# z430/keyword-spotting

Hardware: AMD Instinct MI355X
Metric: 1s 16kHz clips/sec end-to-end (wav->label) (higher is better)
Workload: dtype f32

## Files before the change

### keyword-spotting_amd/csrc/kws_mfcc.hip

```cpp
#include <cstdlib>

#include "kws_augment_dev.h"
#include "kws_internal.h"
#include "kws_mfcc_dev.h"

namespace kws {
namespace {

template <typename T, bool TAIL6>
__device__ __forceinline__ void mfcc_body(const FrontendParams& p, const FrontendTables& t, const T* __restrict__ wav,
                                          float* __restrict__ out, const RefineList& rl) {
    extern __shared__ __attribute__((aligned(16))) unsigned char smem[];
    const int nfp = (p.nfilt + 3) & ~3;
    float* dctb = reinterpret_cast<float*>(smem);
    cf* tw2 = reinterpret_cast<cf*>(dctb + ((p.numcep * nfp + 3) & ~3));
    float* ybuf = reinterpret_cast<float*>(tw2 + 64);
    unsigned char* scr0 = reinterpret_cast<unsigned char*>(ybuf + ((p.chunk_samples + 7) & ~7));

    const int tid = threadIdx.x, lane = tid & 63, wv = tid >> 6;
    const int clip = blockIdx.y;
    const int f0 = blockIdx.x * MFCC_FRAMES_PER_WG;
    const T* __restrict__ x = wav + (size_t)clip * p.n_samples;

    const int s0 = f0 * p.frame_step;
// ... 76 lines not shown
            }
        } else {
#pragma unroll
            for (int n1 = 0; n1 < 8; ++n1) {
                const int i = 64 * n1 + lane;
                const bool in = i < p.frame_len;
                const float la = ya[i], lb = yb[i];
                const float a = in ? la : 0.f, b = (in && has_b) ? lb : 0.f;
                v[n1] = cf{a, b};
                ora |= __builtin_bit_cast(uint32_t, a);
                orb |= __builtin_bit_cast(uint32_t, b);
            }
        }
        const bool nza = __any((ora << 1) != 0u);
        const bool nzb = __any((orb << 1) != 0u);
        const uint32_t flags = mfcc_pair(v, nza, nzb, has_b, p, sc, t1, ml, lane,
                                         out + ((size_t)clip * p.num_frames + fa) * p.numcep,
                                         out + ((size_t)clip * p.num_frames + fa + 1) * p.numcep);
        if (flags && rl.ctr && lane == 0) {
            const unsigned long long old = atomicAdd(reinterpret_cast<unsigned long long*>(rl.ctr), 1ull | ((unsigned long long)__builtin_popcount(flags) << 32));
            const int at = (int)(unsigned)old;
            if (at < rl.cap) rl.list[at] = (int)((((unsigned)(rl.clip0 + clip) * (unsigned)((p.num_frames + 1) / 2) + (unsigned)(fa >> 1)) << 2) | flags);
        }
        wave_lds_order();
    }
}

#ifndef KWS_MFCC_EU
#define KWS_MFCC_EU 4
#endif
__global__ __launch_bounds__(MFCC_THREADS) __attribute__((amdgpu_waves_per_eu(KWS_MFCC_EU, KWS_MFCC_EU))) void kws_mfcc_i16_tile_kernel(FrontendParams p, FrontendTables t,
                                                                    const int16_t* __restrict__ wav,
                                                                    float* __restrict__ out, RefineList rl) {
    mfcc_body<int16_t, true>(p, t, wav, out, rl);
}
__global__ __launch_bounds__(MFCC_THREADS) __attribute__((amdgpu_waves_per_eu(KWS_MFCC_EU, KWS_MFCC_EU))) void kws_mfcc_f32_kernel(FrontendParams p, FrontendTables t,
                                                                    const float* __restrict__ wav,
                                                                    float* __restrict__ out, RefineList rl) {
    mfcc_body<float, true>(p, t, wav, out, rl);
}
__global__ __launch_bounds__(MFCC_THREADS) __attribute__((amdgpu_waves_per_eu(KWS_MFCC_EU, KWS_MFCC_EU))) void kws_mfcc_i16_any_kernel(FrontendParams p, FrontendTables t,
                                                                    const int16_t* __restrict__ wav,
                                                                    float* __restrict__ out, RefineList rl) {
    mfcc_body<int16_t, false>(p, t, wav, out, rl);
}
__global__ __launch_bounds__(MFCC_THREADS) __attribute__((amdgpu_waves_per_eu(KWS_MFCC_EU, KWS_MFCC_EU))) void kws_mfcc_f32_any_kernel(FrontendParams p, FrontendTables t,
                                                                    const float* __restrict__ wav,
                                                                    float* __restrict__ out, RefineList rl) {
    mfcc_body<float, false>(p, t, wav, out, rl);
}

constexpr int WR_PAIRS = 2, WR_FRAMES = 2 * WR_PAIRS;
constexpr int WR_SPAN = 1024;
constexpr int WR_WAVE_BYTES = WR_SPAN * 4 + SCR_BYTES;

typedef float float4_a4 __attribute__((ext_vector_type(4), aligned(4)));
__device__ __forceinline__ void aug_vec8(const AugClip& c, int n0, int n, float (&a)[8]) {
    if (n0 + 8 > n) {
#pragma unroll
        for (int i = 0; i < 8; ++i) a[i] = 0.f;
        return;
    }
    const int r = uniform_i(-c.shift & 7);
    const int base = n0 - c.shift - r;
    uint4 lo = make_uint4(0, 0, 0, 0), hi = lo;
    if (!c.silence) {
        if (base >= 0 && base + 8 <= n) lo = *reinterpret_cast<const uint4*>(c.x + base);
        if (base + 8 >= 0 && base + 16 <= n) hi = *reinterpret_cast<const uint4*>(c.x + base + 8);
    }
    const uint32_t w[8] = {lo.x, lo.y, lo.z, lo.w, hi.x, hi.y, hi.z, hi.w};
    const uint32_t m2 = (r & 4) ? ~0u : 0u, m1 = (r & 2) ? ~0u : 0u;
    uint32_t u[6], v[5];
#pragma unroll
    for (int k = 0; k < 6; ++k) u[k] = (w[k + 2] & m2) | (w[k] & ~m2);
#pragma unroll
    for (int k = 0; k < 5; ++k) v[k] = (u[k + 1] & m1) | (u[k] & ~m1);
#pragma unroll
    for (int k = 0; k < 4; ++k) {
        const uint32_t wd = (r & 1) ? __builtin_amdgcn_alignbyte(v[k + 1], v[k], 2) : v[k];
        a[2 * k] = pcm_unit((int16_t)(wd & 0xffffu));
        a[2 * k + 1] = pcm_unit((int16_t)(wd >> 16));
    }
    if (c.bg) {
        const int k0 = c.off + n0;
        float g[8];
        if (k0 >= 0 && k0 + 8 <= c.bg_len) {
            const float4_a4 g0 = *reinterpret_cast<const float4_a4*>(c.bg + k0);
            const float4_a4 g1 = *reinterpret_cast<const float4_a4*>(c.bg + k0 + 4);
            g[0] = g0.x, g[1] = g0.y, g[2] = g0.z, g[3] = g0.w, g[4] = g1.x, g[5] = g1.y, g[6] = g1.z, g[7] = g1.w;
        } else {
#pragma unroll
            for (int i = 0; i < 8; ++i) {
                const int k = c.off + n0 + i;
                g[i] = (k >= 0 && k < c.bg_len) ? c.bg[k] : 0.f;
            }
        }
#pragma unroll
        for (int i = 0; i < 8; ++i) a[i] = __fadd_rn(a[i], __fmul_rn(g[i], c.vol));
    }
}

__host__ __device__ inline size_t mfcc_wr_lds_bytes(const FrontendParams& p) {
    const int nfp = (p.nfilt + 3) & ~3;
    return sizeof(float) * (size_t)(((p.numcep * nfp + 3) & ~3) + 2 * 64) + (size_t)MFCC_WAVES * WR_WAVE_BYTES;
}

template <bool AUG>
__device__ __forceinline__ void mfcc_wr_body(FrontendParams p, FrontendTables t, const int16_t* __restrict__ wav,
                                             float* __restrict__ out, RefineList rl, int B, int chunks_per_wave,
                                             AugmentArgs aug) {
    extern __shared__ __attribute__((aligned(16))) unsigned char smem[];
    const int nfp = (p.nfilt + 3) & ~3;
    float* dctb = reinterpret_cast<float*>(smem);
    cf* tw2 = reinterpret_cast<cf*>(dctb + ((p.numcep * nfp + 3) & ~3));
    const int tid = threadIdx.x, lane = tid & 63, wv = tid >> 6;
    unsigned char* mine = reinterpret_cast<unsigned char*>(tw2 + 64) + wv * WR_WAVE_BYTES;
    float* ybuf = reinterpret_cast<float*>(mine);
    unsigned char* scr = mine + WR_SPAN * 4;

    for (int i = tid; i < (p.numcep * nfp + 3) / 4; i += MFCC_THREADS)
        reinterpret_cast<float4*>(dctb)[i] = reinterpret_cast<const float4*>(t.dct_pad)[i];
    fill_tw2(t.twiddle, tw2, tid);
    cf t1[8];
    load_twiddles(t.twiddle, lane, t1);
    MelLane ml;
    load_mel_lane(t, lane, ml);
    zero_scratch(scr, lane);

    const int n_chunks = (p.num_frames + WR_FRAMES - 1) / WR_FRAMES;
    const int waves_per_clip = (n_chunks + chunks_per_wave - 1) / chunks_per_wave;
    const int gw = blockIdx.x * MFCC_WAVES + wv;
    const int clip = gw / waves_per_clip, part = gw - clip * waves_per_clip;
    int c = part * chunks_per_wave;
    const int c_end = min(n_chunks, c + chunks_per_wave);
    const bool active = clip < B && c < c_end;
    const int16_t* __restrict__ x = AUG ? nullptr : wav + (size_t)(active ? clip : 0) * p.n_samples;
    AugClip ac{};
    if constexpr (AUG) ac = aug_clip(aug, active ? clip : 0, p.n_samples);
    const int chunk_step = WR_FRAMES * p.frame_step;

    uint4 v0 = make_uint4(0, 0, 0, 0), v1 = v0;
    int16_t before = 0;
    auto fetch = [&](int cc) {
        const int s0 = cc * chunk_step;
        const int n0 = s0 + 8 * lane, n1 = n0 + 512;
        v0 = n0 + 8 <= p.n_samples ? *reinterpret_cast<const uint4*>(x + n0) : make_uint4(0, 0, 0, 0);
        v1 = n1 + 8 <= p.n_samples ? *reinterpret_cast<const uint4*>(x + n1) : make_uint4(0, 0, 0, 0);
        before = s0 > 0 ? x[s0 - 1] : (int16_t)0;
    };
    (void)fetch;
#ifdef KWS_X_MFCC_PREFETCH
    if (!AUG && active) fetch(c);
#endif
    __syncthreads();
    if (!active) return;

    const PairScratch sc = {reinterpret_cast<cf*>(scr + SCR_XBUF), reinterpret_cast<float2*>(scr + SCR_PBUF),
                            reinterpret_cast<float*>(scr + SCR_LBUF), dctb, tw2, nfp};
    const float pre = p.preemph;
    uint32_t fmask = 0u;
    int pair0 = 2 * c;
#define KWS_FLUSH_FLAGS()                                                                                                          \
    if (fmask && rl.ctr) {                                                                                                          \
        const int lane = (int)__builtin_amdgcn_mbcnt_hi(~0u, __builtin_amdgcn_mbcnt_lo(~0u, 0u));  \
        const uint32_t fk = lane < 16 ? (fmask >> (2 * lane)) & 3u : 0u;                                                            \
        const uint32_t has = (uint32_t)__ballot(fk != 0u);                                                                          \
        unsigned long long old = 0ull;                                                                                              \
        if (lane == 0)                                                                                                              \
            old = atomicAdd(reinterpret_cast<unsigned long long*>(rl.ctr),                                                          \
                            (unsigned long long)__builtin_popcount(has) | ((unsigned long long)__builtin_popcount(fmask) << 32));   \
        const int at = __builtin_amdgcn_readfirstlane((int)(unsigned)old) + __builtin_popcount(has & ((1u << (lane & 31)) - 1u));   \
        if (fk != 0u && at < rl.cap)                                                                                                \
            rl.list[at] = (int)((((unsigned)(rl.clip0 + clip) * (unsigned)((p.num_frames + 1) / 2) + (unsigned)(pair0 + lane)) << 2) | fk); \
    }
    for (; c < c_end; ++c) {
#ifndef KWS_X_MFCC_PREFETCH
        if constexpr (!AUG) fetch(c);
#endif
        if constexpr (AUG) {
            const int s0 = c * chunk_step;
            float a0[8], a1[8];
            aug_vec8(ac, s0 + 8 * lane, p.n_samples, a0);
            aug_vec8(ac, s0 + 512 + 8 * lane, p.n_samples, a1);
            const float w0 = __int_as_float(__builtin_amdgcn_update_dpp(0, __float_as_int(a0[7]), 0x138, 0xf, 0xf, false));
            const float w1 = __int_as_float(__builtin_amdgcn_update_dpp(0, __float_as_int(a1[7]), 0x138, 0xf, 0xf, false));
            const float last0 = __int_as_float(__builtin_amdgcn_readlane(__float_as_int(a0[7]), 63));
            const float before_a = s0 > 0 ? aug_sample(ac, s0 - 1, p.n_samples) : 0.f;
            auto emphasise = [&](const float (&a)[8], float prev, int n, float* dst) {
                float y[8];
#pragma unroll
                for (int i = 0; i < 8; ++i) {
                    y[i] = __fsub_rn(a[i], __fmul_rn(pre, prev));
                    prev = a[i];
                }
                if (n == 0) y[0] = a[0];
                if (n + 8 > p.n_samples) {
#pragma unroll
                    for (int i = 0; i < 8; ++i) y[i] = 0.f;
                }
                reinterpret_cast<float4*>(dst)[0] = make_float4(y[0], y[1], y[2], y[3]);
                reinterpret_cast<float4*>(dst)[1] = make_float4(y[4], y[5], y[6], y[7]);
            };
            emphasise(a0, lane == 0 ? before_a : w0, s0 + 8 * lane, ybuf + 8 * lane);
            emphasise(a1, lane == 0 ? last0 : w1, s0 + 512 + 8 * lane, ybuf + 512 + 8 * lane);
        } else {
            const int s0 = c * chunk_step;
            const uint32_t w0 = (uint32_t)__builtin_amdgcn_update_dpp(0, (int)v0.w, 0x138, 0xf, 0xf, false);
            const uint32_t w1 = (uint32_t)__builtin_amdgcn_update_dpp(0, (int)v1.w, 0x138, 0xf, 0xf, false);
            const uint32_t last0 = (uint32_t)__builtin_amdgcn_readlane((int)v0.w, 63);
            float prev0 = lane == 0 ? to_unit(before) : to_unit((int16_t)(w0 >> 16));
            float prev1 = lane == 0 ? to_unit((int16_t)(last0 >> 16)) : to_unit((int16_t)(w1 >> 16));
            auto convert = [&](const uint4& raw, float prev, int n, float* dst) {
                const uint32_t wd[4] = {raw.x, raw.y, raw.z, raw.w};
                float y[8];
#pragma unroll
                for (int i = 0; i < 8; ++i) {
                    const float cur = to_unit((int16_t)((wd[i >> 1] >> (16 * (i & 1))) & 0xffffu));
                    y[i] = __fsub_rn(cur, __fmul_rn(pre, prev));
                    prev = cur;
                }
                if (n == 0) y[0] = to_unit((int16_t)(wd[0] & 0xffffu));
                if (n + 8 > p.n_samples) {
#pragma unroll
                    for (int i = 0; i < 8; ++i) y[i] = 0.f;
                }
                reinterpret_cast<float4*>(dst)[0] = make_float4(y[0], y[1], y[2], y[3]);
                reinterpret_cast<float4*>(dst)[1] = make_float4(y[4], y[5], y[6], y[7]);
            };
            convert(v0, prev0, s0 + 8 * lane, ybuf + 8 * lane);
            convert(v1, prev1, s0 + 512 + 8 * lane, ybuf + 512 + 8 * lane);
        }
        wave_lds_order();
#ifdef KWS_X_MFCC_PREFETCH
        if (!AUG && c + 1 < c_end) fetch(c + 1);
#endif
#pragma unroll 1
        for (int pr = 0; pr < WR_PAIRS; ++pr) {
            const int fa = WR_FRAMES * c + 2 * pr;
            if (fa >= p.num_frames) break;
            const bool has_b = fa + 1 < p.num_frames;
            const float* ya = ybuf + (2 * pr) * p.frame_step;
            const float* yb = ya + p.frame_step;
            cf v[8];
            uint32_t ora = 0u, orb = 0u;
#pragma unroll
            for (int n1 = 0; n1 < 7; ++n1) {
                const int i = 64 * n1 + lane;
                float a = ya[i], b = yb[i];
                if (n1 == 6) {
                    const bool in = i < p.frame_len;
                    a = in ? a : 0.f, b = in ? b : 0.f;
                }
                v[n1] = cf{a, b};
                ora |= __builtin_bit_cast(uint32_t, a);
                orb |= __builtin_bit_cast(uint32_t, b);
            }
            v[7] = cf{0.f, 0.f};
            if (!has_b) {
#pragma unroll
                for (int n1 = 0; n1 < 7; ++n1) v[n1].y = 0.f;
                orb = 0u;
            }
            const bool nza = __any((ora << 1) != 0u);
            const bool nzb = __any((orb << 1) != 0u);
            const uint32_t flags = mfcc_pair(v, nza, nzb, has_b, p, sc, t1, ml, lane,
                                             out + ((size_t)clip * p.num_frames + fa) * p.numcep,
                                             out + ((size_t)clip * p.num_frames + fa + 1) * p.numcep);
            fmask |= flags << (2 * ((fa >> 1) - pair0));
            wave_lds_order();
        }
        if (2 * (c + 1) - pair0 >= 16) {
            KWS_FLUSH_FLAGS()
            fmask = 0u;
            pair0 = 2 * (c + 1);
        }
    }
    KWS_FLUSH_FLAGS()
#undef KWS_FLUSH_FLAGS
}

__global__ __launch_bounds__(MFCC_THREADS) __attribute__((amdgpu_waves_per_eu(KWS_MFCC_EU, KWS_MFCC_EU))) void kws_mfcc_i16_kernel(
    FrontendParams p, FrontendTables t, const int16_t* __restrict__ wav, float* __restrict__ out, RefineList rl, int B, int chunks_per_wave) {
    mfcc_wr_body<false>(p, t, wav, out, rl, B, chunks_per_wave, AugmentArgs{});
}
#ifndef KWS_MFCC_AUG_EU
#define KWS_MFCC_AUG_EU 4
#endif
__global__ __launch_bounds__(MFCC_THREADS) __attribute__((amdgpu_waves_per_eu(KWS_MFCC_AUG_EU, KWS_MFCC_AUG_EU))) void kws_mfcc_augment_i16_kernel(
    FrontendParams p, FrontendTables t, AugmentArgs aug, float* __restrict__ out, RefineList rl, int B, int chunks_per_wave) {
    mfcc_wr_body<true>(p, t, nullptr, out, rl, B, chunks_per_wave, aug);
}

__global__ void kws_preemphasis_f32_kernel(const float* __restrict__ in, int n, float coeff, float* __restrict__ out) {
    for (int i = blockIdx.x * blockDim.x + threadIdx.x; i < n; i += gridDim.x * blockDim.x)
        out[i] = (i > 0) ? __fsub_rn(in[i], __fmul_rn(coeff, in[i - 1])) : in[i];
}

__global__ void kws_framesig_f32_kernel(const float* __restrict__ in, int n, int frame_len, int frame_step,
                                        int num_frames, const float* __restrict__ window,
                                        float* __restrict__ frames) {
    const long total = (long)num_frames * frame_len;
    for (long idx = blockIdx.x * (long)blockDim.x + threadIdx.x; idx < total; idx += (long)gridDim.x * blockDim.x) {
        const int f = (int)(idx / frame_len), i = (int)(idx % frame_len);
        const long s = (long)f * frame_step + i;
        float v = (s < n) ? in[s] : 0.f;
        if (window) v *= window[i];
        frames[idx] = v;
    }
}

__global__ __launch_bounds__(64) void kws_spec512_f32_kernel(FrontendTables t, const float* __restrict__ frames,
                                                             int num_frames, int frame_len, int power,
                                                             float* __restrict__ spec) {
    __shared__ __attribute__((aligned(16))) unsigned char smem[SCR_BYTES + 512];
    cf* xbuf = reinterpret_cast<cf*>(smem + SCR_XBUF);
    float2* pbuf = reinterpret_cast<float2*>(smem + SCR_PBUF);
    cf* tw2 = reinterpret_cast<cf*>(smem + SCR_BYTES);
    const int lane = threadIdx.x;
    const int fa = 2 * blockIdx.x;
    const bool has_b = fa + 1 < num_frames;
    cf t1[8];
    load_twiddles(t.twiddle, lane, t1);
    fill_tw2(t.twiddle, tw2, lane);
    wave_lds_order();
    const float* ya = frames + (size_t)fa * frame_len;
    const float* yb = ya + frame_len;
    cf v[8];
    bool nza = false, nzb = false;
#pragma unroll
    for (int n1 = 0; n1 < 8; ++n1) {
        const int i = 64 * n1 + lane;
        const bool in = i < frame_len;
        v[n1].x = in ? ya[i] : 0.f;
        v[n1].y = (in && has_b) ? yb[i] : 0.f;
        nza |= v[n1].x != 0.f;
        nzb |= v[n1].y != 0.f;
    }
    nza = __any(nza);
    nzb = __any(nzb);
    const PairLevel lv = equalise_levels(v);
    fft512(v, xbuf, t1, tw2, lane);
    float ea, eb;
    const int ident[4] = {lane, lane + 64, lane + 128, lane + 192};
// ... 70 lines not shown
    float vol = 0.f;
    if (d.n_files > 0 && (d.use_background || sil)) {
        const int k = draw_below(w[1], d.n_files);
        const int room = d.bg_len[k] - d.n_samples;
        off = d.bg_start[k] + (room > 0 ? draw_below(w[2], room) : 0);
        const float u = draw_unit(w[3]);
        if (sil)
            vol = u;
        else if (u < d.bg_frequency)
            vol = __fmul_rn(__fdiv_rn(u, d.bg_frequency), d.bg_volume);
    }
    d.bg_off[b] = off;
    d.bg_vol[b] = vol;
    d.silence[b] = sil ? 1 : 0;
}

}

hipError_t launch_augment_draw(hipStream_t s, const DrawArgs& d, int B) {
    hipLaunchKernelGGL(kws_augment_draw_kernel, dim3((B + 255) / 256), dim3(256), 0, s, d, B);
    return hipGetLastError();
}

size_t mfcc_lds_bytes(const FrontendParams& p) {
    const int nfp = (p.nfilt + 3) & ~3;
    return sizeof(float) * (size_t)(((p.numcep * nfp + 3) & ~3) + 2 * 64 + ((p.chunk_samples + 7) & ~7)) +
           (size_t)MFCC_WAVES * SCR_BYTES;
}

template <typename T, typename K>
static hipError_t launch_mfcc_t(K kernel, hipStream_t s, const FrontendParams& p, const FrontendTables& t, const T* d_wav,
                                int B, float* d_out, RefineList rl) {
    dim3 grid((p.num_frames + MFCC_FRAMES_PER_WG - 1) / MFCC_FRAMES_PER_WG, B);
    const size_t lds = mfcc_lds_bytes(p);
    if (lds > 64 * 1024) {
        hipError_t e = hipFuncSetAttribute(reinterpret_cast<const void*>(kernel), hipFuncAttributeMaxDynamicSharedMemorySize, (int)lds);
        if (e != hipSuccess) return e;
    }
    for (int b0 = 0; b0 < B; b0 += 65535) {
        const int nb = (B - b0 < 65535) ? (B - b0) : 65535;
        grid.y = nb;
        rl.clip0 = b0;
        hipLaunchKernelGGL(kernel, grid, dim3(MFCC_THREADS), lds, s, p, t, d_wav + (size_t)b0 * p.n_samples,
                           d_out + (size_t)b0 * p.num_frames * p.numcep, rl);
    }
    return hipGetLastError();
}

bool mfcc_wave_resident_ok(const FrontendParams& p) {
    const bool tail6 = p.frame_len > 384 && p.frame_len <= 448;
    return tail6 && p.vec_ok && (WR_FRAMES * p.frame_step) % 8 == 0 && (WR_FRAMES - 1) * p.frame_step + 448 <= WR_SPAN;
}

static int mfcc_wr_chunks_per_wave(int nb, int n_chunks) {
    int wpc = (n_chunks + 2) / 5;
    wpc = wpc < 1 ? 1 : wpc;
    int cpw = (n_chunks + wpc - 1) / wpc;
    const int fill = (int)(((long)nb * n_chunks + 4095) / 4096);
    cpw = cpw > fill ? (fill < 1 ? 1 : fill) : cpw;
    static const int cpw_env = [] {
        const char* e = getenv("KWS_X_MFCC_CPW");
        return e ? atoi(e) : 0;
    }();
    if (cpw_env > 0) cpw = cpw_env > 16 ? 16 : cpw_env;
    return cpw;
}

hipError_t launch_mfcc_flag(hipStream_t s, const FrontendParams& p, const FrontendTables& t, const int16_t* d_wav, int B,
                            float* d_out, const RefineList& rl) {
    const bool tail6 = p.frame_len > 384 && p.frame_len <= 448;
#ifndef KWS_X_MFCC_TILE_KERNEL
    if (mfcc_wave_resident_ok(p)) {
        const size_t lds = mfcc_wr_lds_bytes(p);
        const int n_chunks = (p.num_frames + WR_FRAMES - 1) / WR_FRAMES;
        for (int b0 = 0; b0 < B; b0 += (1 << 20)) {
            const int nb = B - b0 < (1 << 20) ? B - b0 : (1 << 20);
            const int cpw = mfcc_wr_chunks_per_wave(nb, n_chunks);
            const int waves_per_clip = (n_chunks + cpw - 1) / cpw;
            const long waves = (long)nb * waves_per_clip;
            RefineList r = rl;
            r.clip0 = b0;
            hipLaunchKernelGGL(kws_mfcc_i16_kernel, dim3((unsigned)((waves + MFCC_WAVES - 1) / MFCC_WAVES)), dim3(MFCC_THREADS), lds, s, p, t,
                               d_wav + (size_t)b0 * p.n_samples, d_out + (size_t)b0 * p.num_frames * p.numcep, r, nb, cpw);
        }
        return hipGetLastError();
    }
#endif
    return launch_mfcc_t(tail6 ? kws_mfcc_i16_tile_kernel : kws_mfcc_i16_any_kernel, s, p, t, d_wav, B, d_out, rl);
}

hipError_t launch_mfcc_augment_flag(hipStream_t s, const FrontendParams& p, const FrontendTables& t, const AugmentArgs& a, int B,
                                    float* d_out, const RefineList& rl) {
    if (!mfcc_wave_resident_ok(p)) return hipErrorInvalidValue;
    const size_t lds = mfcc_wr_lds_bytes(p);
    const int n_chunks = (p.num_frames + WR_FRAMES - 1) / WR_FRAMES;
    for (int b0 = 0; b0 < B; b0 += (1 << 20)) {
        const int nb = B - b0 < (1 << 20) ? B - b0 : (1 << 20);
        const int cpw = mfcc_wr_chunks_per_wave(nb, n_chunks);
        const int waves_per_clip = (n_chunks + cpw - 1) / cpw;
        const long waves = (long)nb * waves_per_clip;
        RefineList r = rl;
        r.clip0 = b0;
        AugmentArgs ab = a;
        ab.index += b0;
        if (ab.shift) ab.shift += b0;
        if (ab.bg_off) ab.bg_off += b0;
        if (ab.bg_vol) ab.bg_vol += b0;
        if (ab.silence) ab.silence += b0;
        hipLaunchKernelGGL(kws_mfcc_augment_i16_kernel, dim3((unsigned)((waves + MFCC_WAVES - 1) / MFCC_WAVES)), dim3(MFCC_THREADS), lds, s, p,
                           t, ab, d_out + (size_t)b0 * p.num_frames * p.numcep, r, nb, cpw);
    }
    return hipGetLastError();
}
hipError_t launch_mfcc_f32_flag(hipStream_t s, const FrontendParams& p, const FrontendTables& t, const float* d_wav, int B,
                                float* d_out, const RefineList& rl) {
    const bool tail6 = p.frame_len > 384 && p.frame_len <= 448;
    return launch_mfcc_t(tail6 ? kws_mfcc_f32_kernel : kws_mfcc_f32_any_kernel, s, p, t, d_wav, B, d_out, rl);
}
hipError_t launch_mfcc(hipStream_t s, const FrontendParams& p, const FrontendTables& t, const int16_t* d_wav, int B,
                       float* d_out) {
    return launch_mfcc_flag(s, p, t, d_wav, B, d_out, RefineList{});
}
hipError_t launch_mfcc_f32(hipStream_t s, const FrontendParams& p, const FrontendTables& t, const float* d_wav, int B,
                           float* d_out) {
    return launch_mfcc_f32_flag(s, p, t, d_wav, B, d_out, RefineList{});
}

hipError_t launch_stream_frame(hipStream_t s, const FrontendParams& p, const FrontendTables& t, const int16_t* d_hop,
                               int n_streams, int16_t* d_pcm_ring, int ring_len, float* d_feat_ring, int* d_hops, int* d_refine_ctr) {
    const size_t lds = stream_frame_lds_bytes(p);
    hipLaunchKernelGGL(kws_stream_frame_kernel, dim3((n_streams + 1) / 2), dim3(64), lds, s, p, t, d_hop, n_streams,
                       d_pcm_ring, ring_len, d_feat_ring, d_hops, d_refine_ctr);
    return hipGetLastError();
}

// ... 39 lines not shown
```

### keyword-spotting_amd/csrc/kws_mfcc_dev.h

```cpp
#pragma once
#include "kws_internal.h"
#include "kws_mfcc_f64_dev.h"

namespace kws {
namespace {

typedef float cf __attribute__((ext_vector_type(2)));

__device__ __forceinline__ cf cadd(cf a, cf b) { return a + b; }
__device__ __forceinline__ cf csub(cf a, cf b) { return a - b; }
__device__ __forceinline__ cf cmul(cf a, cf b) {
    cf t, r;
    asm("v_pk_mul_f32 %0, %1, %2 op_sel:[1,1] op_sel_hi:[1,0] neg_lo:[0,1]" : "=v"(t) : "v"(a), "v"(b));
    asm("v_pk_fma_f32 %0, %1, %2, %3 op_sel_hi:[0,1,1]" : "=v"(r) : "v"(a), "v"(b), "v"(t));
    return r;
}
__device__ __forceinline__ cf add_mi(cf a, cf b) {
    cf r;
    asm("v_pk_add_f32 %0, %1, %2 op_sel:[0,1] op_sel_hi:[1,0] neg_hi:[0,1]" : "=v"(r) : "v"(a), "v"(b));
    return r;
}
__device__ __forceinline__ cf sub_mi(cf a, cf b) {
    cf r;
    asm("v_pk_add_f32 %0, %1, %2 op_sel:[0,1] op_sel_hi:[1,0] neg_lo:[0,1]" : "=v"(r) : "v"(a), "v"(b));
// ... 335 lines not shown
        KWS_DPP_STEP("row_shr:2 row_mask:0xf bank_mask:0xf bound_ctrl:1")
        KWS_DPP_STEP("row_shr:4 row_mask:0xf bank_mask:0xf bound_ctrl:1")
        KWS_DPP_STEP("row_shr:8 row_mask:0xf bank_mask:0xf bound_ctrl:1")
        KWS_DPP_STEP("row_bcast:15 row_mask:0xa bank_mask:0xf")
        KWS_DPP_STEP("row_bcast:31 row_mask:0xc bank_mask:0xf")
        "s_nop 0"
        : "+v"(a), "+v"(b), "+v"(ma), "+v"(mb));
#undef KWS_DPP_STEP
    a = __builtin_bit_cast(float, __builtin_amdgcn_readlane(__builtin_bit_cast(int, a), 63));
    b = __builtin_bit_cast(float, __builtin_amdgcn_readlane(__builtin_bit_cast(int, b), 63));
    ma = __builtin_bit_cast(float, __builtin_amdgcn_readlane(__builtin_bit_cast(int, ma), 63));
    mb = __builtin_bit_cast(float, __builtin_amdgcn_readlane(__builtin_bit_cast(int, mb), 63));
}

template <bool FULL>
__device__ __forceinline__ unsigned long long peak_over(float v, float lim) {
    float mn = v;
#define KWS_MM_STEP(ctrl)                                      \
    "v_min_f32_dpp %0, %0, %0 " ctrl "\n\t"                    \
    "s_nop 1\n\t"
    asm("s_nop 1\n\t"
        KWS_MM_STEP("row_shr:1 row_mask:0xf bank_mask:0xf")
        KWS_MM_STEP("row_shr:2 row_mask:0xf bank_mask:0xf")
        KWS_MM_STEP("row_shr:4 row_mask:0xf bank_mask:0xf")
        KWS_MM_STEP("row_shr:8 row_mask:0xf bank_mask:0xf")
        "v_min_f32_dpp %0, %0, %0 row_bcast:15 row_mask:0xa bank_mask:0xf"
        : "+v"(mn));
    if constexpr (FULL)
        asm("s_nop 1\n\t"
            "v_min_f32_dpp %0, %0, %0 row_bcast:31 row_mask:0xc bank_mask:0xf"
            : "+v"(mn));
#undef KWS_MM_STEP
    return __ballot(mn < lim);
}
__device__ __forceinline__ void peak_over2(float va, float vb, float lim_a, float lim_b, bool& over_a, bool& over_b) {
    float a = va, b = vb;
#define KWS_MM_STEP(ctrl)                                      \
    "v_min_f32_dpp %0, %0, %0 " ctrl "\n\t"                    \
    "v_min_f32_dpp %1, %1, %1 " ctrl "\n\t"                    \
    "s_nop 0\n\t"
    asm("s_nop 1\n\t"
        KWS_MM_STEP("row_shr:1 row_mask:0xf bank_mask:0xf")
        KWS_MM_STEP("row_shr:2 row_mask:0xf bank_mask:0xf")
        KWS_MM_STEP("row_shr:4 row_mask:0xf bank_mask:0xf")
        KWS_MM_STEP("row_shr:8 row_mask:0xf bank_mask:0xf")
        KWS_MM_STEP("row_bcast:15 row_mask:0xa bank_mask:0xf")
        KWS_MM_STEP("row_bcast:31 row_mask:0xc bank_mask:0xf")
        : "+v"(a), "+v"(b));
#undef KWS_MM_STEP
    over_a = (__ballot(a < lim_a) >> 63) & 1ull;
    over_b = (__ballot(b < lim_b) >> 63) & 1ull;
}

__device__ __forceinline__ uint32_t mfcc_pair(cf (&v)[8], bool nza, bool nzb, bool has_b, const FrontendParams& p,
                                          const PairScratch& sc, const cf (&t1)[8], const MelLane& ml, int lane,
                                          float* __restrict__ out_a, float* __restrict__ out_b,
                                          float* lds_out_a = nullptr) {
    cf* xbuf = sc.xbuf;
    float2* pbuf = sc.pbuf;
    float* lbuf = sc.lbuf;
    const float* dctb = sc.dctb;
    const cf* tw2 = sc.tw2;
    const uint32_t gth = ml.gth;
    const int nfp = sc.nfp;
    const PairLevel lv = equalise_levels(v);
#if !defined(KWS_X_MFCC_STOP) || KWS_X_MFCC_STOP >= 1
    fft512(v, xbuf, t1, tw2, lane);
#endif
#if defined(KWS_X_MFCC_STOP) && KWS_X_MFCC_STOP <= 1
    if (lane < p.numcep) out_a[lane] = v[0].x + v[1].y + v[2].x + v[3].y + v[4].x + v[5].y + v[6].x + v[7].y + lv.pow_a;
    return 0u;
#endif

    float ea, eb, pka = 0.f, pkb = 0.f;
    if (p.refine_span > 0.f) {
        split_power(v, xbuf, pbuf, lane, 1, nza, nzb, ml.pslot, -1, lv, ea, eb, &pka, &pkb);
        wave_sum2_max2(ea, eb, pka, pkb);
    } else {
        split_power(v, xbuf, pbuf, lane, 1, nza, nzb, ml.pslot, -1, lv, ea, eb);
        wave_sum2(ea, eb);
    }
#if defined(KWS_X_MFCC_STOP) && KWS_X_MFCC_STOP == 2
    if (lane < p.numcep) out_a[lane] = ea + eb + pbuf[lane].x;
    return 0u;
#endif

    float ra = 0.f, fa_ = 0.f, rb = 0.f, fb_ = 0.f;
    {
        const float4* pc = reinterpret_cast<const float4*>(pbuf + lane * MEL_STRIDE);
#pragma unroll
        for (int h = 0; h < MEL_CHUNK / 2; ++h) {
            const float4 pw = pc[h];
            ra = fmaf(ml.rw[2 * h], pw.x, ra);
            fa_ = fmaf(ml.fw[2 * h], pw.x, fa_);
            rb = fmaf(ml.rw[2 * h], pw.y, rb);
            fb_ = fmaf(ml.fw[2 * h], pw.y, fb_);
            ra = fmaf(ml.rw[2 * h + 1], pw.z, ra);
            fa_ = fmaf(ml.fw[2 * h + 1], pw.z, fa_);
            rb = fmaf(ml.rw[2 * h + 1], pw.w, rb);
            fb_ = fmaf(ml.fw[2 * h + 1], pw.w, fb_);
        }
    }
    segment_suffix_sums(ra, fa_, rb, fb_, ml);
    float ma, mb;
    uint32_t flags = 0u;
    {
        const int r0 = gth & 255, nr = (gth >> 8) & 255, q0 = (gth >> 16) & 255, nq = gth >> 24;
        const float gra = __builtin_bit_cast(float, __builtin_amdgcn_ds_bpermute(4 * r0, __builtin_bit_cast(int, ra)));
        const float grb = __builtin_bit_cast(float, __builtin_amdgcn_ds_bpermute(4 * r0, __builtin_bit_cast(int, rb)));
        const float gfa = __builtin_bit_cast(float, __builtin_amdgcn_ds_bpermute(4 * q0, __builtin_bit_cast(int, fa_)));
        const float gfb = __builtin_bit_cast(float, __builtin_amdgcn_ds_bpermute(4 * q0, __builtin_bit_cast(int, fb_)));
        const float sa = (nr ? gra : 0.f) + (nq ? gfa : 0.f);
        const float sb = (nr ? grb : 0.f) + (nq ? gfb : 0.f);
        if (p.nfilt <= 32) {
            const auto sw = __builtin_amdgcn_permlane32_swap(__builtin_bit_cast(unsigned, sa), __builtin_bit_cast(unsigned, sb), false, false);
            const float s = __builtin_bit_cast(float, (unsigned)sw[0]);
            const float l = logf(s == 0.f ? PSF_EPS : s);
            ma = __builtin_bit_cast(float, __builtin_amdgcn_readlane(__builtin_bit_cast(int, l), 0));
            mb = __builtin_bit_cast(float, __builtin_amdgcn_readlane(__builtin_bit_cast(int, l), 32));
#if defined(KWS_X_MFCC_STOP) && KWS_X_MFCC_STOP == 3
            if (lane < p.numcep) out_a[lane] = l + ea + eb;
            return 0u;
#endif
            const int f = lane >> 5, j = lane & 31;
            const float cv = j < p.nfilt ? l - (f ? mb : ma) : 0.f;
            lbuf[64 * f + j] = cv;
            if (p.refine_span > 0.f) {
                const float lim = 0.6931471806f * __builtin_amdgcn_logf(f ? pkb : pka) - (f ? mb : ma) - p.refine_span;
                const unsigned long long over = peak_over<false>(cv, lim);
                flags = (uint32_t)((over >> 31) & 1u) | ((uint32_t)((over >> 63) & 1u) << 1);
            }
        } else {
            const float la = logf(sa == 0.f ? PSF_EPS : sa), lb = logf(sb == 0.f ? PSF_EPS : sb);
            ma = __builtin_bit_cast(float, __builtin_amdgcn_readfirstlane(__builtin_bit_cast(int, la)));
            mb = __builtin_bit_cast(float, __builtin_amdgcn_readfirstlane(__builtin_bit_cast(int, lb)));
            const float cva = lane < p.nfilt ? la - ma : 0.f, cvb = lane < p.nfilt ? lb - mb : 0.f;
            lbuf[lane] = cva;
            lbuf[64 + lane] = cvb;
            if (p.refine_span > 0.f) {
                bool oa, ob;
                peak_over2(cva, cvb, 0.6931471806f * __builtin_amdgcn_logf(pka) - ma - p.refine_span, 0.6931471806f * __builtin_amdgcn_logf(pkb) - mb - p.refine_span, oa, ob);
                flags = (uint32_t)oa | ((uint32_t)ob << 1);
            }
        }
    }
    wave_lds_order();

    {
        const int f = lane >> 5, i = lane & 31;
        if (i < p.numcep && (f == 0 || has_b)) {
            const float4* L4 = reinterpret_cast<const float4*>(lbuf + 64 * f);
            const float4* D4 = reinterpret_cast<const float4*>(dctb + i * nfp);
            float acc = 0.f;
            if (nfp == 28) {
#pragma unroll
                for (int j0 = 0; j0 < 7; j0 += 4) {
                    float4 d[4], l[4];
#pragma unroll
                    for (int j = 0; j < 4; ++j)
                        if (j0 + j < 7) d[j] = D4[j0 + j], l[j] = L4[j0 + j];
#pragma unroll
                    for (int j = 0; j < 4; ++j)
                        if (j0 + j < 7) {
                            acc = fmaf(d[j].x, l[j].x, acc);
                            acc = fmaf(d[j].y, l[j].y, acc);
                            acc = fmaf(d[j].z, l[j].z, acc);
                            acc = fmaf(d[j].w, l[j].w, acc);
                        }
                    __builtin_amdgcn_sched_barrier(0);
                }
            } else {
                for (int j = 0; j < nfp / 4; ++j) {
                    const float4 d = D4[j], l = L4[j];
                    acc = fmaf(d.x, l.x, acc);
                    acc = fmaf(d.y, l.y, acc);
                    acc = fmaf(d.z, l.z, acc);
                    acc = fmaf(d.w, l.w, acc);
                }
            }
            if (i == 0) {
                if (p.append_energy) {
                    const float e = f ? eb : ea;
                    acc = logf(e == 0.f ? PSF_EPS : e);
                } else {
                    float dsum = 0.f;
                    for (int j = 0; j < p.nfilt; ++j) dsum += dctb[j];
                    acc = fmaf(f ? mb : ma, dsum, acc);
                }
            }
            (f ? out_b : out_a)[i] = acc;
            if (lds_out_a && f == 0) lds_out_a[i] = acc;
        }
    }
    wave_lds_order();
    return has_b ? flags : (flags & 1u);
}


constexpr int STREAM_F64_BYTES = 16 * NFFT + 8 * 128;
__host__ __device__ __forceinline__ size_t stream_frame_lds_bytes(const FrontendParams& p) {
    const int nfp = (p.nfilt + 3) & ~3;
    return sizeof(float) * (size_t)(((p.numcep * nfp + 3) & ~3) + 2 * 64) + SCR_BYTES + STREAM_F64_BYTES;
}

template <typename F>
__device__ __forceinline__ void f64_redo_frame(const FrontendParams& p, const FrontendTables& t, d2* X, double* L, F&& get,
                                               float* __restrict__ out, float* lds_out, int lane) {
    bool nz = false;
#pragma unroll
    for (int n1 = 0; n1 < 8; ++n1) {
        const int i = 64 * n1 + lane;
        const float y = i < p.frame_len ? get(i) : 0.f;
        nz |= y != 0.f;
        X[sw512(i)] = d2{(double)y, 0.0};
    }
    nz = __any(nz);
    wave_order();
    spectrum_pair<true, NFFT>(X, X, reinterpret_cast<const d2*>(t.tw64), NFFT, 9, p.frame_len, 1.0 / (double)NFFT, lane);
    const F64Tabs tb = {reinterpret_cast<const d2*>(t.tw64), t.mel_w64, t.dct64, t.mel_edges};
    f64_tail<NBINS>(p, tb, NBINS, X, L, nz, false, false, out, out, lds_out, lane);
}
__device__ __forceinline__ long stream_frame_wave(const FrontendParams& p, const FrontendTables& t,
                                                  const int16_t* __restrict__ hop, int sa, int sb, bool has_b,
                                                  int16_t* __restrict__ pcm_ring, int ring_len,
                                                  float* __restrict__ feat_ring, int hops, unsigned char* smem, int lane,
                                                  float* lds_out_a, int* refine_ctr = nullptr) {
    const int nfp = (p.nfilt + 3) & ~3;
    float* dctb = reinterpret_cast<float*>(smem);
    cf* tw2 = reinterpret_cast<cf*>(dctb + ((p.numcep * nfp + 3) & ~3));
    unsigned char* scr = reinterpret_cast<unsigned char*>(tw2 + 64);
    const int step = p.frame_step;
    const long base = (long)step * hops;

    {
        const int n4 = (p.numcep * nfp + 3) / 4;
        const float4* src = reinterpret_cast<const float4*>(t.dct_pad);
        for (int i0 = 0; i0 < n4; i0 += 128) {
            const int i = i0 + lane, j = i + 64;
            const float4 a = i < n4 ? src[i] : make_float4(0.f, 0.f, 0.f, 0.f);
// ... 113 lines not shown
```

Measured before the change: 7.082 million.

## Specialise MFCC kernel for reference geometry and add optional global-to-LDS chunk DMA

Adds a REF template specialisation that hardcodes frame length, step, filter count and cepstral count for the standard 400/160/26/10 geometry, chosen at launch by a host check. This lets the compiler fold constants and drop runtime branches. It also adds an asynchronous global_load_lds prefetch path that pulls the next chunk's PCM into LDS while the current pair is computed. That path is compiled only when KWS_X_MFCC_CHUNK_DMA is defined, so by default only the specialisation runs. The per-wave LDS buffer layout changes, which may affect occupancy.

```diff
diff --git a/keyword-spotting_amd/csrc/kws_mfcc.hip b/keyword-spotting_amd/csrc/kws_mfcc.hip
--- a/keyword-spotting_amd/csrc/kws_mfcc.hip
+++ b/keyword-spotting_amd/csrc/kws_mfcc.hip
@@ -152,7 +152,20 @@
 
 constexpr int WR_PAIRS = 2, WR_FRAMES = 2 * WR_PAIRS;
 constexpr int WR_SPAN = 1024;
-constexpr int WR_WAVE_BYTES = WR_SPAN * 4 + SCR_BYTES;
+constexpr int WR_DMA_V1_BYTE = 3712, WR_DMA_V1_LANES = 46;
+constexpr int WR_YBUF_BYTES = WR_DMA_V1_BYTE + 16 * WR_DMA_V1_LANES;
+constexpr int WR_WAVE_BYTES = WR_YBUF_BYTES + SCR_BYTES;
+static_assert(WR_YBUF_BYTES >= WR_SPAN * 4, "the converted span (two float4 pairs per lane) lies inside the span buffer");
+static_assert(WR_DMA_V1_BYTE % 16 == 0 && WR_YBUF_BYTES % 16 == 0 && WR_WAVE_BYTES % 16 == 0 && SCR_BYTES % 16 == 0,
+              "both DMA regions and the scratch behind them start on 16 bytes in every wavefront");
+static_assert(WR_DMA_V1_BYTE + 16 * 64 <= WR_WAVE_BYTES, "the 16-byte read-back of every lane stays inside the wavefront's own LDS");
+static_assert(4 * (10 * 28 + 2 * 64) + MFCC_WAVES * WR_WAVE_BYTES <= 40960, "four workgroups per CU at the reference geometry (160 KiB of LDS)");
+
+__device__ __forceinline__ void glds16(const void* base, uint32_t byte_off, uint32_t lds_base) {
+    uint32_t keep;
+    asm volatile("s_nop 4\n\ts_mov_b32 %0, m0\n\ts_mov_b32 m0, %3\n\ts_nop 0\n\tglobal_load_lds_dwordx4 %1, %2\n\ts_mov_b32 m0, %0"
+                 : "=&s"(keep) : "v"(byte_off), "s"(base), "s"(lds_base) : "memory");
+}
 
 typedef float float4_a4 __attribute__((ext_vector_type(4), aligned(4)));
 __device__ __forceinline__ void aug_vec8(const AugClip& c, int n0, int n, float (&a)[8]) {
@@ -205,20 +218,20 @@
     return sizeof(float) * (size_t)(((p.numcep * nfp + 3) & ~3) + 2 * 64) + (size_t)MFCC_WAVES * WR_WAVE_BYTES;
 }
 
-template <bool AUG>
+template <bool AUG, bool REF>
 __device__ __forceinline__ void mfcc_wr_body(FrontendParams p, FrontendTables t, const int16_t* __restrict__ wav,
                                              float* __restrict__ out, RefineList rl, int B, int chunks_per_wave,
                                              AugmentArgs aug) {
     extern __shared__ __attribute__((aligned(16))) unsigned char smem[];
-    const int nfp = (p.nfilt + 3) & ~3;
+    const int nfp = REF ? 28 : (p.nfilt + 3) & ~3, dct_floats = REF ? 10 * 28 : p.numcep * nfp;
     float* dctb = reinterpret_cast<float*>(smem);
-    cf* tw2 = reinterpret_cast<cf*>(dctb + ((p.numcep * nfp + 3) & ~3));
-    const int tid = threadIdx.x, lane = tid & 63, wv = tid >> 6;
+    cf* tw2 = reinterpret_cast<cf*>(dctb + ((dct_floats + 3) & ~3));
+    const int tid = threadIdx.x, lane = tid & 63, wv = AUG ? tid >> 6 : __builtin_amdgcn_readfirstlane(tid >> 6);
     unsigned char* mine = reinterpret_cast<unsigned char*>(tw2 + 64) + wv * WR_WAVE_BYTES;
     float* ybuf = reinterpret_cast<float*>(mine);
-    unsigned char* scr = mine + WR_SPAN * 4;
-
-    for (int i = tid; i < (p.numcep * nfp + 3) / 4; i += MFCC_THREADS)
+    unsigned char* scr = mine + WR_YBUF_BYTES;
+
+    for (int i = tid; i < (dct_floats + 3) / 4; i += MFCC_THREADS)
         reinterpret_cast<float4*>(dctb)[i] = reinterpret_cast<const float4*>(t.dct_pad)[i];
     fill_tw2(t.twiddle, tw2, tid);
     cf t1[8];
@@ -234,10 +247,21 @@
     int c = part * chunks_per_wave;
     const int c_end = min(n_chunks, c + chunks_per_wave);
     const bool active = clip < B && c < c_end;
+#ifdef KWS_X_MFCC_HOT_PCM
+    const int16_t* __restrict__ x = wav;
+#else
     const int16_t* __restrict__ x = AUG ? nullptr : wav + (size_t)(active ? clip : 0) * p.n_samples;
+#endif
     AugClip ac{};
     if constexpr (AUG) ac = aug_clip(aug, active ? clip : 0, p.n_samples);
-    const int chunk_step = WR_FRAMES * p.frame_step;
+    const int frame_step = REF ? 160 : p.frame_step, frame_len = REF ? 400 : p.frame_len;
+    const int chunk_step = WR_FRAMES * frame_step;
+#if !defined(KWS_X_MFCC_CHUNK_DMA) || defined(KWS_X_MFCC_PREFETCH)
+    const bool dma = false;
+#else
+    const bool dma = !AUG && (REF || (8 * frame_step >= 16 * 64 && 4 * (3 * frame_step + 448) <= WR_DMA_V1_BYTE &&
+                                      3 * frame_step + frame_len <= 512 + 8 * WR_DMA_V1_LANES));
+#endif
 
     uint4 v0 = make_uint4(0, 0, 0, 0), v1 = v0;
     int16_t before = 0;
@@ -249,6 +273,27 @@
         before = s0 > 0 ? x[s0 - 1] : (int16_t)0;
     };
     (void)fetch;
+    const int c_first = c;
+    int16_t carried = 0;
+    auto dma_issue = [&](int cc) {
+        const int s0 = cc * chunk_step;
+        const int n0 = s0 + 8 * lane, n1 = n0 + 512;
+        const uint32_t base = (uint32_t)__builtin_amdgcn_readfirstlane((int)lds_addr(mine));
+#ifndef KWS_X_MFCC_DMA_DRY
+        if (n0 + 8 <= p.n_samples) glds16(x, 2u * (uint32_t)n0, base);
+        if (lane < WR_DMA_V1_LANES && n1 + 8 <= p.n_samples) glds16(x, 2u * (uint32_t)n1, base + WR_DMA_V1_BYTE);
+#endif
+    };
+    auto dma_take = [&](int cc) {
+        const int s0 = cc * chunk_step;
+        const int n0 = s0 + 8 * lane, n1 = n0 + 512;
+        asm volatile("s_waitcnt vmcnt(0)" ::: "memory");
+        const uint4 r0 = *reinterpret_cast<const uint4*>(mine + 16 * lane);
+        const uint4 r1 = *reinterpret_cast<const uint4*>(mine + WR_DMA_V1_BYTE + 16 * lane);
+        v0 = n0 + 8 <= p.n_samples ? r0 : make_uint4(0, 0, 0, 0);
+        v1 = lane < WR_DMA_V1_LANES && n1 + 8 <= p.n_samples ? r1 : make_uint4(0, 0, 0, 0);
+        before = carried;
+    };
 #ifdef KWS_X_MFCC_PREFETCH
     if (!AUG && active) fetch(c);
 #endif
@@ -275,7 +320,10 @@
     }
     for (; c < c_end; ++c) {
 #ifndef KWS_X_MFCC_PREFETCH
-        if constexpr (!AUG) fetch(c);
+        if constexpr (!AUG) {
+            if (dma && c != c_first) dma_take(c);
+            else fetch(c);
+        }
 #endif
         if constexpr (AUG) {
             const int s0 = c * chunk_step;
@@ -327,6 +375,7 @@
                 reinterpret_cast<float4*>(dst)[0] = make_float4(y[0], y[1], y[2], y[3]);
                 reinterpret_cast<float4*>(dst)[1] = make_float4(y[4], y[5], y[6], y[7]);
             };
+            if (dma) carried = (int16_t)((uint32_t)__builtin_amdgcn_readlane((int)v1.w, 15) >> 16);
             convert(v0, prev0, s0 + 8 * lane, ybuf + 8 * lane);
             convert(v1, prev1, s0 + 512 + 8 * lane, ybuf + 512 + 8 * lane);
         }
@@ -339,8 +388,8 @@
             const int fa = WR_FRAMES * c + 2 * pr;
             if (fa >= p.num_frames) break;
             const bool has_b = fa + 1 < p.num_frames;
-            const float* ya = ybuf + (2 * pr) * p.frame_step;
-            const float* yb = ya + p.frame_step;
+            const float* ya = ybuf + (2 * pr) * frame_step;
+            const float* yb = ya + frame_step;
             cf v[8];
             uint32_t ora = 0u, orb = 0u;
 #pragma unroll
@@ -348,7 +397,7 @@
                 const int i = 64 * n1 + lane;
                 float a = ya[i], b = yb[i];
                 if (n1 == 6) {
-                    const bool in = i < p.frame_len;
+                    const bool in = i < frame_len;
                     a = in ? a : 0.f, b = in ? b : 0.f;
                 }
                 v[n1] = cf{a, b};
@@ -363,11 +412,13 @@
             }
             const bool nza = __any((ora << 1) != 0u);
             const bool nzb = __any((orb << 1) != 0u);
-            const uint32_t flags = mfcc_pair(v, nza, nzb, has_b, p, sc, t1, ml, lane,
-                                             out + ((size_t)clip * p.num_frames + fa) * p.numcep,
-                                             out + ((size_t)clip * p.num_frames + fa + 1) * p.numcep);
+            const int numcep = REF ? 10 : p.numcep;
+            const uint32_t flags = mfcc_pair<REF>(v, nza, nzb, has_b, p, sc, t1, ml, lane,
+                                                  out + ((size_t)clip * p.num_frames + fa) * numcep,
+                                                  out + ((size_t)clip * p.num_frames + fa + 1) * numcep);
             fmask |= flags << (2 * ((fa >> 1) - pair0));
             wave_lds_order();
+            if (!AUG && dma && pr == 0 && c + 1 < c_end) dma_issue(c + 1);
         }
         if (2 * (c + 1) - pair0 >= 16) {
             KWS_FLUSH_FLAGS()
@@ -381,14 +432,18 @@
 
 __global__ __launch_bounds__(MFCC_THREADS) __attribute__((amdgpu_waves_per_eu(KWS_MFCC_EU, KWS_MFCC_EU))) void kws_mfcc_i16_kernel(
     FrontendParams p, FrontendTables t, const int16_t* __restrict__ wav, float* __restrict__ out, RefineList rl, int B, int chunks_per_wave) {
-    mfcc_wr_body<false>(p, t, wav, out, rl, B, chunks_per_wave, AugmentArgs{});
+    mfcc_wr_body<false, true>(p, t, wav, out, rl, B, chunks_per_wave, AugmentArgs{});
+}
+__global__ __launch_bounds__(MFCC_THREADS) __attribute__((amdgpu_waves_per_eu(KWS_MFCC_EU, KWS_MFCC_EU))) void kws_mfcc_i16_general_kernel(
+    FrontendParams p, FrontendTables t, const int16_t* __restrict__ wav, float* __restrict__ out, RefineList rl, int B, int chunks_per_wave) {
+    mfcc_wr_body<false, false>(p, t, wav, out, rl, B, chunks_per_wave, AugmentArgs{});
 }
 #ifndef KWS_MFCC_AUG_EU
 #define KWS_MFCC_AUG_EU 4
 #endif
 __global__ __launch_bounds__(MFCC_THREADS) __attribute__((amdgpu_waves_per_eu(KWS_MFCC_AUG_EU, KWS_MFCC_AUG_EU))) void kws_mfcc_augment_i16_kernel(
     FrontendParams p, FrontendTables t, AugmentArgs aug, float* __restrict__ out, RefineList rl, int B, int chunks_per_wave) {
-    mfcc_wr_body<true>(p, t, nullptr, out, rl, B, chunks_per_wave, aug);
+    mfcc_wr_body<true, false>(p, t, nullptr, out, rl, B, chunks_per_wave, aug);
 }
 
 __global__ void kws_preemphasis_f32_kernel(const float* __restrict__ in, int n, float coeff, float* __restrict__ out) {
@@ -565,6 +620,13 @@
     return tail6 && p.vec_ok && (WR_FRAMES * p.frame_step) % 8 == 0 && (WR_FRAMES - 1) * p.frame_step + 448 <= WR_SPAN;
 }
 
+static bool mfcc_wr_ref_geometry(const FrontendParams& p) {
+#ifdef KWS_X_MFCC_NO_REF
+    return false;
+#endif
+    return p.frame_len == 400 && p.frame_step == 160 && p.nfilt == 26 && p.numcep == 10 && p.append_energy && p.refine_span > 0.f;
+}
+
 static int mfcc_wr_chunks_per_wave(int nb, int n_chunks) {
     int wpc = (n_chunks + 2) / 5;
     wpc = wpc < 1 ? 1 : wpc;
@@ -593,7 +655,8 @@
             const long waves = (long)nb * waves_per_clip;
             RefineList r = rl;
             r.clip0 = b0;
-            hipLaunchKernelGGL(kws_mfcc_i16_kernel, dim3((unsigned)((waves + MFCC_WAVES - 1) / MFCC_WAVES)), dim3(MFCC_THREADS), lds, s, p, t,
+            hipLaunchKernelGGL(mfcc_wr_ref_geometry(p) ? kws_mfcc_i16_kernel : kws_mfcc_i16_general_kernel,
+                               dim3((unsigned)((waves + MFCC_WAVES - 1) / MFCC_WAVES)), dim3(MFCC_THREADS), lds, s, p, t,
                                d_wav + (size_t)b0 * p.n_samples, d_out + (size_t)b0 * p.num_frames * p.numcep, r, nb, cpw);
         }
         return hipGetLastError();
diff --git a/keyword-spotting_amd/csrc/kws_mfcc_dev.h b/keyword-spotting_amd/csrc/kws_mfcc_dev.h
--- a/keyword-spotting_amd/csrc/kws_mfcc_dev.h
+++ b/keyword-spotting_amd/csrc/kws_mfcc_dev.h
@@ -411,6 +411,7 @@
     over_b = (__ballot(b < lim_b) >> 63) & 1ull;
 }
 
+template <bool REF = false>
 __device__ __forceinline__ uint32_t mfcc_pair(cf (&v)[8], bool nza, bool nzb, bool has_b, const FrontendParams& p,
                                           const PairScratch& sc, const cf (&t1)[8], const MelLane& ml, int lane,
                                           float* __restrict__ out_a, float* __restrict__ out_b,
@@ -421,18 +422,20 @@
     const float* dctb = sc.dctb;
     const cf* tw2 = sc.tw2;
     const uint32_t gth = ml.gth;
-    const int nfp = sc.nfp;
+    const int nfp = REF ? 28 : sc.nfp;
+    const int nfilt = REF ? 26 : p.nfilt, numcep = REF ? 10 : p.numcep;
+    const bool refine = REF || p.refine_span > 0.f;
     const PairLevel lv = equalise_levels(v);
 #if !defined(KWS_X_MFCC_STOP) || KWS_X_MFCC_STOP >= 1
     fft512(v, xbuf, t1, tw2, lane);
 #endif
 #if defined(KWS_X_MFCC_STOP) && KWS_X_MFCC_STOP <= 1
-    if (lane < p.numcep) out_a[lane] = v[0].x + v[1].y + v[2].x + v[3].y + v[4].x + v[5].y + v[6].x + v[7].y + lv.pow_a;
+    if (lane < numcep) out_a[lane] = v[0].x + v[1].y + v[2].x + v[3].y + v[4].x + v[5].y + v[6].x + v[7].y + lv.pow_a;
     return 0u;
 #endif
 
     float ea, eb, pka = 0.f, pkb = 0.f;
-    if (p.refine_span > 0.f) {
+    if (refine) {
         split_power(v, xbuf, pbuf, lane, 1, nza, nzb, ml.pslot, -1, lv, ea, eb, &pka, &pkb);
         wave_sum2_max2(ea, eb, pka, pkb);
     } else {
@@ -440,7 +443,7 @@
         wave_sum2(ea, eb);
     }
 #if defined(KWS_X_MFCC_STOP) && KWS_X_MFCC_STOP == 2
-    if (lane < p.numcep) out_a[lane] = ea + eb + pbuf[lane].x;
+    if (lane < numcep) out_a[lane] = ea + eb + pbuf[lane].x;
     return 0u;
 #endif
 
@@ -471,20 +474,20 @@
         const float gfb = __builtin_bit_cast(float, __builtin_amdgcn_ds_bpermute(4 * q0, __builtin_bit_cast(int, fb_)));
         const float sa = (nr ? gra : 0.f) + (nq ? gfa : 0.f);
         const float sb = (nr ? grb : 0.f) + (nq ? gfb : 0.f);
-        if (p.nfilt <= 32) {
+        if (REF || nfilt <= 32) {
             const auto sw = __builtin_amdgcn_permlane32_swap(__builtin_bit_cast(unsigned, sa), __builtin_bit_cast(unsigned, sb), false, false);
             const float s = __builtin_bit_cast(float, (unsigned)sw[0]);
             const float l = logf(s == 0.f ? PSF_EPS : s);
             ma = __builtin_bit_cast(float, __builtin_amdgcn_readlane(__builtin_bit_cast(int, l), 0));
             mb = __builtin_bit_cast(float, __builtin_amdgcn_readlane(__builtin_bit_cast(int, l), 32));
 #if defined(KWS_X_MFCC_STOP) && KWS_X_MFCC_STOP == 3
-            if (lane < p.numcep) out_a[lane] = l + ea + eb;
+            if (lane < numcep) out_a[lane] = l + ea + eb;
             return 0u;
 #endif
             const int f = lane >> 5, j = lane & 31;
-            const float cv = j < p.nfilt ? l - (f ? mb : ma) : 0.f;
+            const float cv = j < nfilt ? l - (f ? mb : ma) : 0.f;
             lbuf[64 * f + j] = cv;
-            if (p.refine_span > 0.f) {
+            if (refine) {
                 const float lim = 0.6931471806f * __builtin_amdgcn_logf(f ? pkb : pka) - (f ? mb : ma) - p.refine_span;
                 const unsigned long long over = peak_over<false>(cv, lim);
                 flags = (uint32_t)((over >> 31) & 1u) | ((uint32_t)((over >> 63) & 1u) << 1);
@@ -493,10 +496,10 @@
             const float la = logf(sa == 0.f ? PSF_EPS : sa), lb = logf(sb == 0.f ? PSF_EPS : sb);
             ma = __builtin_bit_cast(float, __builtin_amdgcn_readfirstlane(__builtin_bit_cast(int, la)));
             mb = __builtin_bit_cast(float, __builtin_amdgcn_readfirstlane(__builtin_bit_cast(int, lb)));
-            const float cva = lane < p.nfilt ? la - ma : 0.f, cvb = lane < p.nfilt ? lb - mb : 0.f;
+            const float cva = lane < nfilt ? la - ma : 0.f, cvb = lane < nfilt ? lb - mb : 0.f;
             lbuf[lane] = cva;
             lbuf[64 + lane] = cvb;
-            if (p.refine_span > 0.f) {
+            if (refine) {
                 bool oa, ob;
                 peak_over2(cva, cvb, 0.6931471806f * __builtin_amdgcn_logf(pka) - ma - p.refine_span, 0.6931471806f * __builtin_amdgcn_logf(pkb) - mb - p.refine_span, oa, ob);
                 flags = (uint32_t)oa | ((uint32_t)ob << 1);
@@ -507,11 +510,11 @@
 
     {
         const int f = lane >> 5, i = lane & 31;
-        if (i < p.numcep && (f == 0 || has_b)) {
+        if (i < numcep && (f == 0 || has_b)) {
             const float4* L4 = reinterpret_cast<const float4*>(lbuf + 64 * f);
             const float4* D4 = reinterpret_cast<const float4*>(dctb + i * nfp);
             float acc = 0.f;
-            if (nfp == 28) {
+            if (REF || nfp == 28) {
 #pragma unroll
                 for (int j0 = 0; j0 < 7; j0 += 4) {
                     float4 d[4], l[4];
@@ -538,12 +541,12 @@
                 }
             }
             if (i == 0) {
-                if (p.append_energy) {
+                if (REF || p.append_energy) {
                     const float e = f ? eb : ea;
                     acc = logf(e == 0.f ? PSF_EPS : e);
                 } else {
                     float dsum = 0.f;
-                    for (int j = 0; j < p.nfilt; ++j) dsum += dctb[j];
+                    for (int j = 0; j < nfilt; ++j) dsum += dctb[j];
                     acc = fmaf(f ? mb : ma, dsum, acc);
                 }
             }
```

Measured after the change: 7.081 million. No clear change (-0.0%).
